# FastLM/CXL-SpecKV

Hardware: AMD Instinct MI355X
Metric: KV blocks/s fetch+decompress (higher is better)
Workload: dtype fp32 (int8 records -> fp16)

## Files before the change

cxl-speckv_amd/csrc/attend_kv.hip:

```cpp
#include "kernels.hpp"
#include "codec_device.hpp"
#include "attend_device.hpp"

namespace speckv {

namespace {

__device__ __forceinline__ uint2 kv_ldg8(const uint8_t* p)
{
    const u32x2 v = __builtin_nontemporal_load(SPECKV_GP(u32x2, p));
    return make_uint2(v.x, v.y);
}
__device__ __forceinline__ uint32_t kv_ldg1(const uint8_t* p) { return *SPECKV_GP(uint8_t, p); }
__device__ __forceinline__ f32x4 kv_ldg_f4(const float* p) { return *SPECKV_GP(f32x4, p); }

}

__global__ __launch_bounds__(256) __attribute__((amdgpu_waves_per_eu(4, 4))) void k_attend_k8v4(AttendArgs a, const AttendKvSide* __restrict__ vside)
{
    const uint32_t lane = threadIdx.x & 63u;
    const uint32_t wave = __builtin_amdgcn_readfirstlane(threadIdx.x >> 6);
    const uint32_t c = lane & 15u, kb = lane >> 4;
    const uint32_t split = a.rows_first ? blockIdx.y : blockIdx.x, by = a.rows_first ? blockIdx.x : blockIdx.y;
    if (a.rows_first && by >= a.rows_real) return;
    const uint32_t hq = a.heads / 4u;
    uint32_t seq = by / hq;
    if (a.order) seq = a.order[seq];
    const uint32_t head = (by % hq) * 4u + wave;
    const uint64_t row = static_cast<uint64_t>(seq) * a.heads + head;
    const AttendSeq sq = a.seqs[seq];
    if (split >= sq.n_splits) {
        if (sq.n_splits == 0u && split == 0u) attend_zero_rows(a.direct_out, a.direct_lse, a.g, row, lane);
        return;
    }
    const AttendKvSide vsd = vside[seq];
    const uint64_t part = sq.part_base + static_cast<uint64_t>(head) * sq.n_splits + split;
    const uint32_t n_pages = sq.n_pages;

    uint32_t qd[8];
    float qscale = 1.0f;
    auto quantise_query = [&]() {
        float xq[32];
        float mx = 0.0f;
        const uint16_t* qsrc = a.q16 + (row * a.g + min(c, a.g - 1u)) * 128u + kb * 16u;
#pragma unroll
        for (int i = 0; i < 4; ++i) {
            const uint4 w = *reinterpret_cast<const uint4*>(qsrc + 8 * (i & 1) + 64 * (i >> 1));
            const uint32_t ws[4] = {w.x, w.y, w.z, w.w};
#pragma unroll
            for (int k = 0; k < 8; ++k) {
                xq[8 * i + k] = static_cast<float>(__builtin_bit_cast(_Float16, static_cast<uint16_t>(ws[k >> 1] >> (16 * (k & 1)))));
                mx = fmaxf(mx, fabsf(xq[8 * i + k]));
            }
        }
        mx = max_over_kb(mx);
        const bool finite = mx < INFINITY;
        const float sc = (mx > 0.0f) ? (finite ? div448_of_f16_value(mx) : mx / 448.0f) : 1.0f;
        const float rcp = finite ? rcp_of_scale(sc) : 0.0f;
        const bool live = c < a.g;
#pragma unroll
        for (int i = 0; i < 8; ++i) {
            float v[4];
#pragma unroll
            for (int k = 0; k < 4; ++k) {
                const float x = xq[4 * i + k];
                const float qt = finite ? __builtin_copysignf(div_by_scale(x, sc, rcp), x) : x / sc;
                v[k] = live ? fminf(fmaxf(qt, -448.0f), 448.0f) : 0.0f;
            }
            int pk = __builtin_amdgcn_cvt_pk_fp8_f32(v[0], v[1], 0, false);
            pk = __builtin_amdgcn_cvt_pk_fp8_f32(v[2], v[3], pk, true);
            qd[i] = static_cast<uint32_t>(pk);
        }
        qscale = (live ? sc : 1.0f) * a.scale_log2e;
    };

    const uint32_t n_tiles = (n_pages + 15u) / 16u;
    const uint32_t t0 = split * sq.tiles_per_split;
    const uint32_t t1 = min(t0 + sq.tiles_per_split, n_tiles);
    float m_run = -INFINITY, l_run = 0.0f;
    f32x4 acc[8];
#pragma unroll
    for (int t = 0; t < 8; ++t) acc[t] = f32x4{0.0f, 0.0f, 0.0f, 0.0f};

    if (t0 < t1) {
        const uint8_t* kp = sq.lin_base + sq.k_first * 2048ull + head * 128u + kb * 16u + (static_cast<uint64_t>(t0) * 32u + c) * 1024u;
        const float* kt = sq.scale_tab + (sq.k_first + static_cast<uint64_t>(t0) * 16u) + 4u * kb;
        const uint8_t* vtile = vsd.v_base + ((vsd.v_first >> 4) + t0) * static_cast<uint64_t>(kMx4TileBytes);
        const uint8_t* vp = vtile + 2u * kb * 1024u + head * 128u + 8u * c;
        const uint8_t* vc = vtile + kMx4CodePlane + 2u * kb * 64u + head * 8u + (c >> 1);

        uint4 kx[2][2];
        uint2 vx[4];
        uint32_t vcode[4];
        f32x4 ks4;
        auto issue_k = [&]() {
#pragma unroll
            for (int b = 0; b < 2; ++b) { kx[b][0] = ldg16(kp + 16384 * b); kx[b][1] = ldg16(kp + 16384 * b + 64); }
            ks4 = kv_ldg_f4(kt);
        };
        auto issue_v = [&]() {
#pragma unroll
            for (int r = 0; r < 4; ++r) vx[r] = kv_ldg8(vp + 1024 * (r & 1) + 8192 * (r >> 1));
#pragma unroll
            for (int r = 0; r < 4; ++r) vcode[r] = kv_ldg1(vc + 64 * (r & 1) + 512 * (r >> 1));
        };
        __builtin_amdgcn_sched_barrier(0);
        issue_k();
        __builtin_amdgcn_sched_barrier(0);
        issue_v();
        __builtin_amdgcn_sched_barrier(0);
        quantise_query();
        __builtin_amdgcn_sched_barrier(0);
        const bool ragged = (n_pages & 15u) != 0u;
#pragma unroll 1
        for (uint32_t tile = t0; tile < t1; ++tile) {
            const uint32_t step = (tile + 1u < t1) ? 1u : 0u;
            float sc[8];
#pragma unroll
            for (int b = 0; b < 2; ++b) {
                const uint32_t kd[8] = {kx[b][0].x, kx[b][0].y, kx[b][0].z, kx[b][0].w, kx[b][1].x, kx[b][1].y, kx[b][1].z, kx[b][1].w};
                f32x4 s = {0.0f, 0.0f, 0.0f, 0.0f};
#pragma unroll
                for (int st = 0; st < 4; ++st)
                    s = __builtin_amdgcn_mfma_f32_16x16x32_fp8_fp8(pack64(kd[2 * st], kd[2 * st + 1]), pack64(qd[2 * st], qd[2 * st + 1]), s, 0, 0, 0);
#pragma unroll
                for (int i = 0; i < 4; ++i) sc[4 * b + i] = s[i] * (ks4[2 * b + (i >> 1)] * qscale);
            }
            if (ragged && tile + 1u == n_tiles) {
#pragma unroll
                for (int r = 0; r < 4; ++r) {
                    const uint32_t pg = tile * 16u + 2u * kb + (r & 1) + 8u * (r >> 1);
                    if (pg >= n_pages) { sc[2 * r] = -INFINITY; sc[2 * r + 1] = -INFINITY; vcode[r] = 0u; }
                }
            }
            __builtin_amdgcn_sched_barrier(0);
            kp += step * 32768u; kt += step * 16u;
            issue_k();
            __builtin_amdgcn_sched_barrier(0);
            float mx = sc[0];
#pragma unroll
            for (int j = 1; j < 8; ++j) mx = fmaxf(mx, sc[j]);
            mx = max_over_kb(mx);
            const float m_new = fmaxf(m_run, mx);
            const float m_use = (m_new == -INFINITY) ? 0.0f : m_new;
            const float f = __builtin_amdgcn_exp2f(m_run - m_use);
            m_run = m_new;
            float psum = 0.0f;
            f16x8 P;
#pragma unroll
            for (int j = 0; j < 8; ++j) {
                const float p = __builtin_amdgcn_exp2f(sc[j] - m_use);
                psum += p;
                P[j] = static_cast<_Float16>(p);
            }
            l_run = l_run * f + psum;
            float vsc[4];
#pragma unroll
            for (int r = 0; r < 4; ++r) vsc[r] = __uint_as_float(vcode[r] << 23);
#define KV_PV(T, WORD, SEL)                                                                                                       \
    {                                                                                                                              \
        const u32x4 vw = {__builtin_bit_cast(uint32_t, __builtin_amdgcn_cvt_scalef32_pk_f16_fp4(vx[0].WORD, vsc[0], SEL)),          \
                          __builtin_bit_cast(uint32_t, __builtin_amdgcn_cvt_scalef32_pk_f16_fp4(vx[1].WORD, vsc[1], SEL)),          \
                          __builtin_bit_cast(uint32_t, __builtin_amdgcn_cvt_scalef32_pk_f16_fp4(vx[2].WORD, vsc[2], SEL)),          \
                          __builtin_bit_cast(uint32_t, __builtin_amdgcn_cvt_scalef32_pk_f16_fp4(vx[3].WORD, vsc[3], SEL))};         \
        acc[T] = __builtin_amdgcn_mfma_f32_16x16x32_f16(__builtin_bit_cast(f16x8, vw), P, acc[T] * f, 0, 0, 0);                     \
    }
            KV_PV(0, x, 0) KV_PV(1, x, 1) KV_PV(2, x, 2) KV_PV(3, x, 3) KV_PV(4, y, 0) KV_PV(5, y, 1) KV_PV(6, y, 2) KV_PV(7, y, 3)
#undef KV_PV
            __builtin_amdgcn_sched_barrier(0);
            vp += step * kMx4TileBytes; vc += step * kMx4TileBytes;
            issue_v();
            __builtin_amdgcn_sched_barrier(0);
        }
    }
    const float l_tot = sum_over_kb(l_run);
    if (sq.n_splits == 1u) {
        if (c < a.g) {
            const float w = l_tot > 0.0f ? 1.0f / l_tot : 0.0f;
            float* dst = a.direct_out + (row * a.g + c) * 128u + 32u * kb;
#pragma unroll
            for (int i = 0; i < 4; ++i) {
                *reinterpret_cast<f32x4*>(dst + 8 * i) = f32x4{acc[0][i], acc[1][i], acc[2][i], acc[3][i]} * w;
                *reinterpret_cast<f32x4*>(dst + 8 * i + 4) = f32x4{acc[4][i], acc[5][i], acc[6][i], acc[7][i]} * w;
            }
            if (a.direct_lse && kb == 0)
                a.direct_lse[row * a.g + c] = l_tot > 0.0f ? (m_run + log2f(l_tot)) * 0.6931471805599453f : -INFINITY;
        }
        return;
    }
    if (kb == 0) {
        a.part_ml[part * 32u + c] = m_run;
        a.part_ml[part * 32u + 16u + c] = l_tot;
    }
    if (c < a.g) {
        float* dst = a.part_acc + (part * 16u + c) * 128u + 32u * kb;
#pragma unroll
        for (int i = 0; i < 4; ++i) {
            *reinterpret_cast<f32x4*>(dst + 8 * i) = f32x4{acc[0][i], acc[1][i], acc[2][i], acc[3][i]};
            *reinterpret_cast<f32x4*>(dst + 8 * i + 4) = f32x4{acc[4][i], acc[5][i], acc[6][i], acc[7][i]};
        }
    }
}

hipError_t launch_attend_k8v4(const AttendArgs& a, const AttendKvSide* d_vside, uint32_t n_seq, bool merge, float* d_out, float* d_lse, hipStream_t s)
{
    if (n_seq == 0) return hipSuccess;
    if (!a.seqs || !d_vside || !a.q16 || a.direct_out != d_out || a.heads % 4u || a.g == 0 || a.g > 16u) return hipErrorInvalidValue;
    AttendArgs ar = a;
    const uint32_t rows = n_seq * (a.heads / 4u), splits = a.n_splits ? a.n_splits : 1u;
    ar.rows_real = rows;
    const dim3 gr = a.rows_first ? dim3(rows | 1u, splits) : dim3(splits, rows);
    hipLaunchKernelGGL(k_attend_k8v4, gr, dim3(256), 0, s, ar, d_vside);
    const hipError_t e = hipGetLastError();
    if (e != hipSuccess || !merge) return e;
    return launch_attend_combine(a, n_seq, d_out, d_lse, s);
}

}
```

cxl-speckv_amd/csrc/tuning.cpp:

```cpp
#include "tuning.hpp"

#include <cstdlib>
#include <cstring>
#include <mutex>

namespace speckv {

namespace {
struct Key { const char* name; const char* env; int32_t Tuning::* field; };
const Key kKeys[] = {
    {"attend_splits", "SPECKV_ATTEND_SPLITS", &Tuning::attend_splits},
    {"attend_tiles_per_split", "SPECKV_ATTEND_TILES_PER_SPLIT", &Tuning::attend_tiles_per_split},
    {"attend_general", "SPECKV_ATTEND_GENERAL", &Tuning::attend_general},
    {"attend_fold_launch", "SPECKV_ATTEND_FOLD_LAUNCH", &Tuning::attend_fold_launch},
    {"attend_layers_loop", "SPECKV_ATTEND_LAYERS_LOOP", &Tuning::attend_layers_loop},
    {"attend_fp8_dma", "SPECKV_ATTEND_FP8_DMA", &Tuning::attend_fp8_dma},
    {"attend_fp8_striped_table", "SPECKV_ATTEND_FP8_STRIPED_TABLE", &Tuning::attend_fp8_striped_table},
    {"attend_int4_striped_wg", "SPECKV_ATTEND_INT4_STRIPED_WG", &Tuning::attend_int4_striped_wg},
    {"attend_fp8_table_regs", "SPECKV_ATTEND_FP8_TABLE_REGS", &Tuning::attend_fp8_table_regs},
    {"attend_stream", "SPECKV_ATTEND_STREAM", &Tuning::attend_stream},
    {"attend_mx4_one_half", "SPECKV_ATTEND_MX4_ONE_HALF", &Tuning::attend_mx4_one_half},
    {"attend_order_as_given", "SPECKV_ATTEND_ORDER_AS_GIVEN", &Tuning::attend_order_as_given},
    {"tc_multipass", "SPECKV_TC_MULTIPASS", &Tuning::tc_multipass},
    {"tc_scan", "SPECKV_TC_SCAN", &Tuning::tc_scan},
    {"tc_no_pre", "SPECKV_TC_NO_PRE", &Tuning::tc_no_pre},
    {"tc_no_split_tiles", "SPECKV_TC_NO_SPLIT_TILES", &Tuning::tc_no_split_tiles},
    {"td_one_pass", "SPECKV_TD_ONE_PASS", &Tuning::td_one_pass},
    {"td_expand_per_element", "SPECKV_TD_EXPAND_PER_ELEMENT", &Tuning::td_expand_per_element},
    {"tc_batch_one_wg", "SPECKV_TC_BATCH_ONE_WG", &Tuning::tc_batch_one_wg},
    {"flush_no_small", "SPECKV_FLUSH_NO_SMALL", &Tuning::flush_no_small},
    {"flush_small_words", "SPECKV_FLUSH_SMALL_WORDS", &Tuning::flush_small_words},
    {"predict_batch_path", "SPECKV_PREDICT_BATCH_PATH", &Tuning::predict_batch_path},
    {"wgs_per_cu", "SPECKV_WGS_PER_CU", &Tuning::wgs_per_cu},
    {"rounds_consecutive", "SPECKV_ROUNDS", &Tuning::rounds_consecutive},
    {"remote_engine", "SPECKV_REMOTE_ENGINE", &Tuning::remote_engine},
    {"copy_min_run_kb", "SPECKV_COPY_MIN_RUN_KB", &Tuning::copy_min_run_kb},
    {"slots_kind_fast", "SPECKV_SLOTS_KIND_FAST", &Tuning::slots_kind_fast},
};
int32_t parse(const char* env_name, const char* v)
{
    if (!strcmp(env_name, "SPECKV_TC_SCAN")) return !strcmp(v, "wg") ? 1 : !strcmp(v, "serial") ? 2 : atoi(v);
    if (!strcmp(env_name, "SPECKV_REMOTE_ENGINE")) return !strcmp(v, "kernel") ? 1 : !strcmp(v, "copy") ? 2 : atoi(v);
    if (!strcmp(env_name, "SPECKV_ROUNDS")) return !strcmp(v, "consecutive") ? 1 : atoi(v);
    if (!*v) return 1;
    const int32_t n = static_cast<int32_t>(atoi(v));
    return (n == 0 && v[0] != '0') ? 1 : n;
}
Tuning g_tuning;
std::once_flag g_once;
}

Tuning& tuning()
{
    std::call_once(g_once, [] {
        for (const Key& k : kKeys)
            if (const char* v = getenv(k.env)) g_tuning.*(k.field) = parse(k.env, v);
    });
    return g_tuning;
}

int tuning_set(const char* key, long long value)
{
    if (!key) return -1;
    Tuning& t = tuning();
    for (const Key& k : kKeys)
        if (!strcmp(k.name, key)) { t.*(k.field) = static_cast<int32_t>(value); return 0; }
    return -1;
}

}
```

cxl-speckv_amd/csrc/tuning.hpp:

```cpp
#pragma once
#include <cstdint>

namespace speckv {

struct Tuning {
    int32_t attend_splits = 0;
    int32_t attend_tiles_per_split = 0;
    int32_t attend_stream = 0;
    int32_t attend_mx4_one_half = 0;
    int32_t attend_order_as_given = 0;
    int32_t attend_general = 0;
    int32_t attend_fp8_table_regs = 0;
    int32_t attend_fp8_dma = 0;
    int32_t attend_fp8_striped_table = 0;
    int32_t attend_int4_striped_wg = 0;
    int32_t attend_layers_loop = 0;
    int32_t attend_fold_launch = 0;
    int32_t tc_multipass = 0;
    int32_t tc_scan = 0;
    int32_t tc_no_pre = 0;
    int32_t tc_no_split_tiles = 0;
    int32_t td_one_pass = 0;
    int32_t td_expand_per_element = 0;
    int32_t tc_batch_one_wg = 0;
    int32_t flush_no_small = 0;
    int32_t flush_small_words = 0;
    int32_t predict_batch_path = 0;
    int32_t wgs_per_cu = 0;
    int32_t rounds_consecutive = 0;
    int32_t remote_engine = 0;
    int32_t copy_min_run_kb = 1024;
    int32_t slots_kind_fast = 0;
};

Tuning& tuning();
int tuning_set(const char* key, long long value);

}
```

Before: 773.5 million.

## Add LDS-DMA double-buffered variant of k8v4 attend kernel and make it default

Adds a new k8v4 attention kernel that streams K, V, scales and codes into per-wave LDS buffers using global_load_lds with swizzled layouts, double-buffered two tiles ahead, and reads them back with explicit waitcnt-controlled ds_reads. The intent is to hide global load latency and reduce VGPR pressure from register-held prefetches. Shared math is factored into helper functions reused by both kernels. The default tuning value (0, tested with >=0) selects the new kernel, which lowers occupancy to 3 waves per EU and relies on hand-counted vmcnt values that could be fragile.

```diff
diff --git a/cxl-speckv_amd/csrc/attend_kv.hip b/cxl-speckv_amd/csrc/attend_kv.hip
--- a/cxl-speckv_amd/csrc/attend_kv.hip
+++ b/cxl-speckv_amd/csrc/attend_kv.hip
@@ -1,18 +1,165 @@
 #include "kernels.hpp"
 #include "codec_device.hpp"
 #include "attend_device.hpp"
+#include "tuning.hpp"
 
 namespace speckv {
 
 namespace {
 
-__device__ __forceinline__ uint2 kv_ldg8(const uint8_t* p)
-{
-    const u32x2 v = __builtin_nontemporal_load(SPECKV_GP(u32x2, p));
-    return make_uint2(v.x, v.y);
-}
+__device__ __forceinline__ u32x2 kv_ldg8(const uint8_t* p) { return __builtin_nontemporal_load(SPECKV_GP(u32x2, p)); }
 __device__ __forceinline__ uint32_t kv_ldg1(const uint8_t* p) { return *SPECKV_GP(uint8_t, p); }
 __device__ __forceinline__ f32x4 kv_ldg_f4(const float* p) { return *SPECKV_GP(f32x4, p); }
+
+__device__ __forceinline__ void kv_quantise_rows(const u32x4 (&w4)[4], bool live, uint32_t (&qd)[8], float& row_scale)
+{
+    float xq[32];
+    float mx = 0.0f;
+#pragma unroll
+    for (int i = 0; i < 4; ++i) {
+        const uint32_t ws[4] = {w4[i].x, w4[i].y, w4[i].z, w4[i].w};
+#pragma unroll
+        for (int k = 0; k < 8; ++k) {
+            xq[8 * i + k] = static_cast<float>(__builtin_bit_cast(_Float16, static_cast<uint16_t>(ws[k >> 1] >> (16 * (k & 1)))));
+            mx = fmaxf(mx, fabsf(xq[8 * i + k]));
+        }
+    }
+    mx = max_over_kb(mx);
+    const bool finite = mx < INFINITY;
+    const float sc = (mx > 0.0f) ? (finite ? div448_of_f16_value(mx) : mx / 448.0f) : 1.0f;
+    const float rcp = finite ? rcp_of_scale(sc) : 0.0f;
+#pragma unroll
+    for (int i = 0; i < 8; ++i) {
+        float v[4];
+#pragma unroll
+        for (int k = 0; k < 4; ++k) {
+            const float x = xq[4 * i + k];
+            const float qt = finite ? __builtin_copysignf(div_by_scale(x, sc, rcp), x) : x / sc;
+            v[k] = live ? fminf(fmaxf(qt, -448.0f), 448.0f) : 0.0f;
+        }
+        int pk = __builtin_amdgcn_cvt_pk_fp8_f32(v[0], v[1], 0, false);
+        pk = __builtin_amdgcn_cvt_pk_fp8_f32(v[2], v[3], pk, true);
+        qd[i] = static_cast<uint32_t>(pk);
+    }
+    row_scale = live ? sc : 1.0f;
+}
+
+__device__ __forceinline__ void kv_store(const AttendArgs& a, uint32_t n_splits, uint64_t row, uint64_t part, uint32_t c, uint32_t kb,
+                                         const f32x4 (&acc)[8], float m_run, float l_run)
+{
+    const float l_tot = sum_over_kb(l_run);
+    if (n_splits == 1u) {
+        if (c < a.g) {
+            const float w = l_tot > 0.0f ? 1.0f / l_tot : 0.0f;
+            float* dst = a.direct_out + (row * a.g + c) * 128u + 32u * kb;
+#pragma unroll
+            for (int i = 0; i < 4; ++i) {
+                *reinterpret_cast<f32x4*>(dst + 8 * i) = f32x4{acc[0][i], acc[1][i], acc[2][i], acc[3][i]} * w;
+                *reinterpret_cast<f32x4*>(dst + 8 * i + 4) = f32x4{acc[4][i], acc[5][i], acc[6][i], acc[7][i]} * w;
+            }
+            if (a.direct_lse && kb == 0)
+                a.direct_lse[row * a.g + c] = l_tot > 0.0f ? (m_run + log2f(l_tot)) * 0.6931471805599453f : -INFINITY;
+        }
+        return;
+    }
+    if (kb == 0) {
+        a.part_ml[part * 32u + c] = m_run;
+        a.part_ml[part * 32u + 16u + c] = l_tot;
+    }
+    if (c < a.g) {
+        float* dst = a.part_acc + (part * 16u + c) * 128u + 32u * kb;
+#pragma unroll
+        for (int i = 0; i < 4; ++i) {
+            *reinterpret_cast<f32x4*>(dst + 8 * i) = f32x4{acc[0][i], acc[1][i], acc[2][i], acc[3][i]};
+            *reinterpret_cast<f32x4*>(dst + 8 * i + 4) = f32x4{acc[4][i], acc[5][i], acc[6][i], acc[7][i]};
+        }
+    }
+}
+
+__device__ __forceinline__ void kv_scores(const uint32_t (&kd)[2][8], const uint32_t (&qd)[8], f32x4 ks4, float qscale, float (&sc)[8])
+{
+#pragma unroll
+    for (int b = 0; b < 2; ++b) {
+        f32x4 s = {0.0f, 0.0f, 0.0f, 0.0f};
+#pragma unroll
+        for (int st = 0; st < 4; ++st)
+            s = __builtin_amdgcn_mfma_f32_16x16x32_fp8_fp8(pack64(kd[b][2 * st], kd[b][2 * st + 1]), pack64(qd[2 * st], qd[2 * st + 1]), s, 0, 0, 0);
+#pragma unroll
+        for (int i = 0; i < 4; ++i) sc[4 * b + i] = s[i] * (ks4[2 * b + (i >> 1)] * qscale);
+    }
+}
+__device__ __forceinline__ void kv_mask_pages(uint32_t tile, uint32_t kb, uint32_t n_pages, float (&sc)[8], uint32_t (&vcode)[4])
+{
+#pragma unroll
+    for (int r = 0; r < 4; ++r) {
+        const uint32_t pg = tile * 16u + 2u * kb + (r & 1) + 8u * (r >> 1);
+        if (pg >= n_pages) { sc[2 * r] = -INFINITY; sc[2 * r + 1] = -INFINITY; vcode[r] = 0u; }
+    }
+}
+__device__ __forceinline__ float kv_softmax(const float (&sc)[8], float& m_run, float& l_run, f16x8& P)
+{
+    float mx = sc[0];
+#pragma unroll
+    for (int j = 1; j < 8; ++j) mx = fmaxf(mx, sc[j]);
+    mx = max_over_kb(mx);
+    const float m_new = fmaxf(m_run, mx);
+    const float m_use = (m_new == -INFINITY) ? 0.0f : m_new;
+    const float f = __builtin_amdgcn_exp2f(m_run - m_use);
+    m_run = m_new;
+    float psum = 0.0f;
+#pragma unroll
+    for (int j = 0; j < 8; ++j) {
+        const float p = __builtin_amdgcn_exp2f(sc[j] - m_use);
+        psum += p;
+        P[j] = static_cast<_Float16>(p);
+    }
+    l_run = l_run * f + psum;
+    return f;
+}
+__device__ __forceinline__ void kv_pv(const u32x2 (&vx)[4], const uint32_t (&vcode)[4], f16x8 P, float f, f32x4 (&acc)[8])
+{
+    float vsc[4];
+#pragma unroll
+    for (int r = 0; r < 4; ++r) vsc[r] = __uint_as_float(vcode[r] << 23);
+#define KV_PV(T, WORD, SEL)                                                                                                       \
+    {                                                                                                                              \
+        const u32x4 vw = {__builtin_bit_cast(uint32_t, __builtin_amdgcn_cvt_scalef32_pk_f16_fp4(vx[0].WORD, vsc[0], SEL)),          \
+                          __builtin_bit_cast(uint32_t, __builtin_amdgcn_cvt_scalef32_pk_f16_fp4(vx[1].WORD, vsc[1], SEL)),          \
+                          __builtin_bit_cast(uint32_t, __builtin_amdgcn_cvt_scalef32_pk_f16_fp4(vx[2].WORD, vsc[2], SEL)),          \
+                          __builtin_bit_cast(uint32_t, __builtin_amdgcn_cvt_scalef32_pk_f16_fp4(vx[3].WORD, vsc[3], SEL))};         \
+        acc[T] = __builtin_amdgcn_mfma_f32_16x16x32_f16(__builtin_bit_cast(f16x8, vw), P, acc[T] * f, 0, 0, 0);                     \
+    }
+    KV_PV(0, x, 0) KV_PV(1, x, 1) KV_PV(2, x, 2) KV_PV(3, x, 3) KV_PV(4, y, 0) KV_PV(5, y, 1) KV_PV(6, y, 2) KV_PV(7, y, 3)
+#undef KV_PV
+}
+
+constexpr uint32_t kKdV = 4096u, kKdS = 6144u, kKdC = kKdS + 64u, kKdBuf = 6400u;
+__device__ __forceinline__ uint32_t kd_row_slot(uint32_t r) { return r ^ ((r >> 2) & 1u); }
+__device__ __forceinline__ uint32_t kd_piece_xor(uint32_t r) { return (r >> 1) & 7u; }
+__device__ __forceinline__ uint32_t kd_page_slot(uint32_t p) { return p ^ ((p >> 1) & 1u); }
+__device__ __forceinline__ void kd_dma16_nt(uint32_t lds_dst, const uint8_t* base, uint32_t voff)
+{
+    uint32_t keep;
+    asm volatile("s_mov_b32 %0, m0\n\ts_mov_b32 m0, %1\n\ts_nop 0\n\tglobal_load_lds_dwordx4 %2, %3 nt\n\ts_mov_b32 m0, %0"
+                 : "=&s"(keep) : "s"(lds_dst), "v"(voff), "s"(base) : "memory");
+}
+__device__ __forceinline__ void kd_take_k(uint32_t rd0, uint32_t rd1, uint32_t rs, uint32_t rc, u32x4 (&k)[4], f32x4& ks, uint32_t (&code)[4])
+{
+    asm volatile("s_waitcnt vmcnt(9)\n\t"
+                 "ds_read_b128 %0, %9\n\tds_read_b128 %1, %10\n\tds_read_b128 %2, %9 offset:2048\n\tds_read_b128 %3, %10 offset:2048\n\t"
+                 "ds_read_b128 %4, %11\n\t"
+                 "ds_read_u8 %5, %12\n\tds_read_u8 %6, %12 offset:8\n\tds_read_u8 %7, %12 offset:64\n\tds_read_u8 %8, %12 offset:72\n\t"
+                 "s_waitcnt lgkmcnt(0)"
+                 : "=&v"(k[0]), "=&v"(k[1]), "=&v"(k[2]), "=&v"(k[3]), "=&v"(ks), "=&v"(code[0]), "=&v"(code[1]), "=&v"(code[2]), "=&v"(code[3])
+                 : "v"(rd0), "v"(rd1), "v"(rs), "v"(rc) : "memory");
+}
+__device__ __forceinline__ void kd_take_v(uint32_t rd0, uint32_t rd1, u32x2 (&v)[4])
+{
+    asm volatile("s_waitcnt vmcnt(12)\n\t"
+                 "ds_read_b64 %0, %4\n\tds_read_b64 %1, %5\n\tds_read_b64 %2, %4 offset:1024\n\tds_read_b64 %3, %5 offset:1024\n\t"
+                 "s_waitcnt lgkmcnt(0)"
+                 : "=&v"(v[0]), "=&v"(v[1]), "=&v"(v[2]), "=&v"(v[3]) : "v"(rd0), "v"(rd1) : "memory");
+}
 
 }
 
@@ -40,38 +187,12 @@
     uint32_t qd[8];
     float qscale = 1.0f;
     auto quantise_query = [&]() {
-        float xq[32];
-        float mx = 0.0f;
         const uint16_t* qsrc = a.q16 + (row * a.g + min(c, a.g - 1u)) * 128u + kb * 16u;
-#pragma unroll
-        for (int i = 0; i < 4; ++i) {
-            const uint4 w = *reinterpret_cast<const uint4*>(qsrc + 8 * (i & 1) + 64 * (i >> 1));
-            const uint32_t ws[4] = {w.x, w.y, w.z, w.w};
-#pragma unroll
-            for (int k = 0; k < 8; ++k) {
-                xq[8 * i + k] = static_cast<float>(__builtin_bit_cast(_Float16, static_cast<uint16_t>(ws[k >> 1] >> (16 * (k & 1)))));
-                mx = fmaxf(mx, fabsf(xq[8 * i + k]));
-            }
-        }
-        mx = max_over_kb(mx);
-        const bool finite = mx < INFINITY;
-        const float sc = (mx > 0.0f) ? (finite ? div448_of_f16_value(mx) : mx / 448.0f) : 1.0f;
-        const float rcp = finite ? rcp_of_scale(sc) : 0.0f;
-        const bool live = c < a.g;
-#pragma unroll
-        for (int i = 0; i < 8; ++i) {
-            float v[4];
-#pragma unroll
-            for (int k = 0; k < 4; ++k) {
-                const float x = xq[4 * i + k];
-                const float qt = finite ? __builtin_copysignf(div_by_scale(x, sc, rcp), x) : x / sc;
-                v[k] = live ? fminf(fmaxf(qt, -448.0f), 448.0f) : 0.0f;
-            }
-            int pk = __builtin_amdgcn_cvt_pk_fp8_f32(v[0], v[1], 0, false);
-            pk = __builtin_amdgcn_cvt_pk_fp8_f32(v[2], v[3], pk, true);
-            qd[i] = static_cast<uint32_t>(pk);
-        }
-        qscale = (live ? sc : 1.0f) * a.scale_log2e;
+        u32x4 w4[4];
+#pragma unroll
+        for (int i = 0; i < 4; ++i) w4[i] = *reinterpret_cast<const u32x4*>(qsrc + 8 * (i & 1) + 64 * (i >> 1));
+        kv_quantise_rows(w4, c < a.g, qd, qscale);
+        qscale *= a.scale_log2e;
     };
 
     const uint32_t n_tiles = (n_pages + 15u) / 16u;
@@ -90,7 +211,7 @@
         const uint8_t* vc = vtile + kMx4CodePlane + 2u * kb * 64u + head * 8u + (c >> 1);
 
         uint4 kx[2][2];
-        uint2 vx[4];
+        u32x2 vx[4];
         uint32_t vcode[4];
         f32x4 ks4;
         auto issue_k = [&]() {
@@ -116,90 +237,134 @@
         for (uint32_t tile = t0; tile < t1; ++tile) {
             const uint32_t step = (tile + 1u < t1) ? 1u : 0u;
             float sc[8];
-#pragma unroll
-            for (int b = 0; b < 2; ++b) {
-                const uint32_t kd[8] = {kx[b][0].x, kx[b][0].y, kx[b][0].z, kx[b][0].w, kx[b][1].x, kx[b][1].y, kx[b][1].z, kx[b][1].w};
-                f32x4 s = {0.0f, 0.0f, 0.0f, 0.0f};
-#pragma unroll
-                for (int st = 0; st < 4; ++st)
-                    s = __builtin_amdgcn_mfma_f32_16x16x32_fp8_fp8(pack64(kd[2 * st], kd[2 * st + 1]), pack64(qd[2 * st], qd[2 * st + 1]), s, 0, 0, 0);
-#pragma unroll
-                for (int i = 0; i < 4; ++i) sc[4 * b + i] = s[i] * (ks4[2 * b + (i >> 1)] * qscale);
-            }
-            if (ragged && tile + 1u == n_tiles) {
-#pragma unroll
-                for (int r = 0; r < 4; ++r) {
-                    const uint32_t pg = tile * 16u + 2u * kb + (r & 1) + 8u * (r >> 1);
-                    if (pg >= n_pages) { sc[2 * r] = -INFINITY; sc[2 * r + 1] = -INFINITY; vcode[r] = 0u; }
-                }
-            }
+            const uint32_t kd[2][8] = {{kx[0][0].x, kx[0][0].y, kx[0][0].z, kx[0][0].w, kx[0][1].x, kx[0][1].y, kx[0][1].z, kx[0][1].w},
+                                       {kx[1][0].x, kx[1][0].y, kx[1][0].z, kx[1][0].w, kx[1][1].x, kx[1][1].y, kx[1][1].z, kx[1][1].w}};
+            kv_scores(kd, qd, ks4, qscale, sc);
+            if (ragged && tile + 1u == n_tiles) kv_mask_pages(tile, kb, n_pages, sc, vcode);
             __builtin_amdgcn_sched_barrier(0);
             kp += step * 32768u; kt += step * 16u;
             issue_k();
             __builtin_amdgcn_sched_barrier(0);
-            float mx = sc[0];
-#pragma unroll
-            for (int j = 1; j < 8; ++j) mx = fmaxf(mx, sc[j]);
-            mx = max_over_kb(mx);
-            const float m_new = fmaxf(m_run, mx);
-            const float m_use = (m_new == -INFINITY) ? 0.0f : m_new;
-            const float f = __builtin_amdgcn_exp2f(m_run - m_use);
-            m_run = m_new;
-            float psum = 0.0f;
             f16x8 P;
-#pragma unroll
-            for (int j = 0; j < 8; ++j) {
-                const float p = __builtin_amdgcn_exp2f(sc[j] - m_use);
-                psum += p;
-                P[j] = static_cast<_Float16>(p);
-            }
-            l_run = l_run * f + psum;
-            float vsc[4];
-#pragma unroll
-            for (int r = 0; r < 4; ++r) vsc[r] = __uint_as_float(vcode[r] << 23);
-#define KV_PV(T, WORD, SEL)                                                                                                       \
-    {                                                                                                                              \
-        const u32x4 vw = {__builtin_bit_cast(uint32_t, __builtin_amdgcn_cvt_scalef32_pk_f16_fp4(vx[0].WORD, vsc[0], SEL)),          \
-                          __builtin_bit_cast(uint32_t, __builtin_amdgcn_cvt_scalef32_pk_f16_fp4(vx[1].WORD, vsc[1], SEL)),          \
-                          __builtin_bit_cast(uint32_t, __builtin_amdgcn_cvt_scalef32_pk_f16_fp4(vx[2].WORD, vsc[2], SEL)),          \
-                          __builtin_bit_cast(uint32_t, __builtin_amdgcn_cvt_scalef32_pk_f16_fp4(vx[3].WORD, vsc[3], SEL))};         \
-        acc[T] = __builtin_amdgcn_mfma_f32_16x16x32_f16(__builtin_bit_cast(f16x8, vw), P, acc[T] * f, 0, 0, 0);                     \
-    }
-            KV_PV(0, x, 0) KV_PV(1, x, 1) KV_PV(2, x, 2) KV_PV(3, x, 3) KV_PV(4, y, 0) KV_PV(5, y, 1) KV_PV(6, y, 2) KV_PV(7, y, 3)
-#undef KV_PV
+            const float f = kv_softmax(sc, m_run, l_run, P);
+            kv_pv(vx, vcode, P, f, acc);
             __builtin_amdgcn_sched_barrier(0);
             vp += step * kMx4TileBytes; vc += step * kMx4TileBytes;
             issue_v();
             __builtin_amdgcn_sched_barrier(0);
         }
     }
-    const float l_tot = sum_over_kb(l_run);
-    if (sq.n_splits == 1u) {
-        if (c < a.g) {
-            const float w = l_tot > 0.0f ? 1.0f / l_tot : 0.0f;
-            float* dst = a.direct_out + (row * a.g + c) * 128u + 32u * kb;
-#pragma unroll
-            for (int i = 0; i < 4; ++i) {
-                *reinterpret_cast<f32x4*>(dst + 8 * i) = f32x4{acc[0][i], acc[1][i], acc[2][i], acc[3][i]} * w;
-                *reinterpret_cast<f32x4*>(dst + 8 * i + 4) = f32x4{acc[4][i], acc[5][i], acc[6][i], acc[7][i]} * w;
-            }
-            if (a.direct_lse && kb == 0)
-                a.direct_lse[row * a.g + c] = l_tot > 0.0f ? (m_run + log2f(l_tot)) * 0.6931471805599453f : -INFINITY;
-        }
+    kv_store(a, sq.n_splits, row, part, c, kb, acc, m_run, l_run);
+}
+
+__global__ __launch_bounds__(256) __attribute__((amdgpu_waves_per_eu(3, 3))) void k_attend_k8v4_dma(AttendArgs a, const AttendKvSide* __restrict__ vside)
+{
+    __shared__ __attribute__((aligned(16))) uint8_t lds[4][2 * kKdBuf];
+    const uint32_t lane = threadIdx.x & 63u;
+    const uint32_t wave = __builtin_amdgcn_readfirstlane(threadIdx.x >> 6);
+    const uint32_t c = lane & 15u, kb = lane >> 4;
+    const uint32_t split = a.rows_first ? blockIdx.y : blockIdx.x, by = a.rows_first ? blockIdx.x : blockIdx.y;
+    if (a.rows_first && by >= a.rows_real) return;
+    const uint32_t hq = a.heads / 4u;
+    uint32_t seq = by / hq;
+    if (a.order) seq = a.order[seq];
+    const uint32_t head = (by % hq) * 4u + wave;
+    const uint64_t row = static_cast<uint64_t>(seq) * a.heads + head;
+    const AttendSeq sq = a.seqs[seq];
+    if (split >= sq.n_splits) {
+        if (sq.n_splits == 0u && split == 0u) attend_zero_rows(a.direct_out, a.direct_lse, a.g, row, lane);
         return;
     }
-    if (kb == 0) {
-        a.part_ml[part * 32u + c] = m_run;
-        a.part_ml[part * 32u + 16u + c] = l_tot;
-    }
-    if (c < a.g) {
-        float* dst = a.part_acc + (part * 16u + c) * 128u + 32u * kb;
-#pragma unroll
-        for (int i = 0; i < 4; ++i) {
-            *reinterpret_cast<f32x4*>(dst + 8 * i) = f32x4{acc[0][i], acc[1][i], acc[2][i], acc[3][i]};
-            *reinterpret_cast<f32x4*>(dst + 8 * i + 4) = f32x4{acc[4][i], acc[5][i], acc[6][i], acc[7][i]};
-        }
-    }
+    const AttendKvSide vsd = vside[seq];
+    const uint64_t part = sq.part_base + static_cast<uint64_t>(head) * sq.n_splits + split;
+    const uint32_t n_pages = sq.n_pages;
+    const uint32_t n_tiles = (n_pages + 15u) / 16u;
+    const uint32_t t0 = __builtin_amdgcn_readfirstlane(split * sq.tiles_per_split);
+    const uint32_t t1 = __builtin_amdgcn_readfirstlane(min(t0 + sq.tiles_per_split, n_tiles));
+    float m_run = -INFINITY, l_run = 0.0f;
+    f32x4 acc[8];
+#pragma unroll
+    for (int t = 0; t < 8; ++t) acc[t] = f32x4{0.0f, 0.0f, 0.0f, 0.0f};
+
+    if (t0 < t1) {
+        const uint8_t* kreg = uniform_ptr(sq.lin_base + sq.k_first * 2048ull + head * 128u);
+        const uint8_t* vtile0 = vsd.v_base + (vsd.v_first >> 4) * static_cast<uint64_t>(kMx4TileBytes);
+        const uint8_t* vreg = uniform_ptr(vtile0 + head * 128u);
+        uint32_t gk[4], gv[2];
+#pragma unroll
+        for (uint32_t i = 0; i < 4; ++i) {
+            const uint32_t r = kd_row_slot(8u * i + (lane >> 3));
+            gk[i] = r * 1024u + (((lane & 7u) ^ kd_piece_xor(r)) * 16u);
+        }
+#pragma unroll
+        for (uint32_t i = 0; i < 2; ++i) gv[i] = kd_page_slot(8u * i + (lane >> 3)) * 1024u + (lane & 7u) * 16u;
+        const uint32_t cl = (lane - 16u) & 31u;
+        const uint8_t* sc_src = lane < 16u ? reinterpret_cast<const uint8_t*>(sq.scale_tab + sq.k_first + lane)
+                                           : vtile0 + kMx4CodePlane + (cl >> 1) * 64u + head * 8u + (cl & 1u) * 4u;
+        const uint32_t sc_step = lane < 16u ? 64u : kMx4TileBytes;
+        const uint32_t lbase = __builtin_amdgcn_readfirstlane(static_cast<uint32_t>(reinterpret_cast<uintptr_t>(&lds[wave][0])));
+        const uint32_t last = t1 - 1u;
+        auto issue_k = [&](uint32_t tt, uint32_t buf) {
+            const uint32_t tc = min(tt, last);
+            const uint8_t* src = kreg + static_cast<uint64_t>(tc) * 32768u;
+            const uint32_t dst = lbase + buf * kKdBuf;
+#pragma unroll
+            for (uint32_t i = 0; i < 4; ++i) kd_dma16_nt(dst + 1024u * i, src, gk[i]);
+            if (lane < 48u) dma4v(dst + kKdS, sc_src + static_cast<uint64_t>(tc) * sc_step);
+        };
+        auto issue_v = [&](uint32_t tt, uint32_t buf) {
+            const uint8_t* src = vreg + static_cast<uint64_t>(min(tt, last)) * kMx4TileBytes;
+            const uint32_t dst = lbase + buf * kKdBuf + kKdV;
+#pragma unroll
+            for (uint32_t i = 0; i < 2; ++i) kd_dma16_nt(dst + 1024u * i, src, gv[i]);
+        };
+        const uint32_t kslot = kd_row_slot(c), kxr = kd_piece_xor(c);
+        const uint32_t rdk0 = lbase + kslot * 128u + ((kb ^ kxr) * 16u);
+        const uint32_t rdk1 = lbase + kslot * 128u + (((4u + kb) ^ kxr) * 16u);
+        const uint32_t rsc = lbase + kKdS + kb * 16u;
+        const uint32_t rcd = lbase + kKdC + kb * 16u + (c >> 1);
+        const uint32_t rdv0 = lbase + kKdV + kd_page_slot(2u * kb) * 128u + 8u * c;
+        const uint32_t rdv1 = lbase + kKdV + kd_page_slot(2u * kb + 1u) * 128u + 8u * c;
+        issue_k(t0, 0u);
+        u32x4 qw[4];
+        {
+            const uint16_t* qsrc = a.q16 + (row * a.g + min(c, a.g - 1u)) * 128u + kb * 16u;
+            asm volatile("global_load_dwordx4 %0, %4, off\n\tglobal_load_dwordx4 %1, %4, off offset:16\n\t"
+                         "global_load_dwordx4 %2, %4, off offset:128\n\tglobal_load_dwordx4 %3, %4, off offset:144"
+                         : "=&v"(qw[0]), "=&v"(qw[1]), "=&v"(qw[2]), "=&v"(qw[3]) : "v"(qsrc) : "memory");
+        }
+        issue_v(t0, 0u);
+        issue_k(t0 + 1u, 1u);
+        issue_v(t0 + 1u, 1u);
+        asm volatile("s_waitcnt vmcnt(9)" : "+v"(qw[0]), "+v"(qw[1]), "+v"(qw[2]), "+v"(qw[3]) :: "memory");
+        uint32_t qd[8];
+        float qscale;
+        kv_quantise_rows(qw, c < a.g, qd, qscale);
+        qscale *= a.scale_log2e;
+        const bool ragged = (n_pages & 15u) != 0u;
+#pragma unroll 1
+        for (uint32_t tile = t0; tile < t1; ++tile) {
+            const uint32_t buf = (tile - t0) & 1u, bo = buf * kKdBuf;
+            u32x4 kx[4];
+            f32x4 ks4;
+            uint32_t vcode[4];
+            kd_take_k(rdk0 + bo, rdk1 + bo, rsc + bo, rcd + bo, kx, ks4, vcode);
+            issue_k(tile + 2u, buf);
+            float sc[8];
+            const uint32_t kd[2][8] = {{kx[0].x, kx[0].y, kx[0].z, kx[0].w, kx[1].x, kx[1].y, kx[1].z, kx[1].w},
+                                       {kx[2].x, kx[2].y, kx[2].z, kx[2].w, kx[3].x, kx[3].y, kx[3].z, kx[3].w}};
+            kv_scores(kd, qd, ks4, qscale, sc);
+            if (ragged && tile + 1u == n_tiles) kv_mask_pages(tile, kb, n_pages, sc, vcode);
+            f16x8 P;
+            const float f = kv_softmax(sc, m_run, l_run, P);
+            u32x2 vx[4];
+            kd_take_v(rdv0 + bo, rdv1 + bo, vx);
+            issue_v(tile + 2u, buf);
+            kv_pv(vx, vcode, P, f, acc);
+        }
+        asm volatile("s_waitcnt vmcnt(0)" ::: "memory");
+    }
+    kv_store(a, sq.n_splits, row, part, c, kb, acc, m_run, l_run);
 }
 
 hipError_t launch_attend_k8v4(const AttendArgs& a, const AttendKvSide* d_vside, uint32_t n_seq, bool merge, float* d_out, float* d_lse, hipStream_t s)
@@ -210,7 +375,8 @@
     const uint32_t rows = n_seq * (a.heads / 4u), splits = a.n_splits ? a.n_splits : 1u;
     ar.rows_real = rows;
     const dim3 gr = a.rows_first ? dim3(rows | 1u, splits) : dim3(splits, rows);
-    hipLaunchKernelGGL(k_attend_k8v4, gr, dim3(256), 0, s, ar, d_vside);
+    if (tuning().attend_k8v4_dma >= 0) hipLaunchKernelGGL(k_attend_k8v4_dma, gr, dim3(256), 0, s, ar, d_vside);
+    else hipLaunchKernelGGL(k_attend_k8v4, gr, dim3(256), 0, s, ar, d_vside);
     const hipError_t e = hipGetLastError();
     if (e != hipSuccess || !merge) return e;
     return launch_attend_combine(a, n_seq, d_out, d_lse, s);
diff --git a/cxl-speckv_amd/csrc/tuning.cpp b/cxl-speckv_amd/csrc/tuning.cpp
--- a/cxl-speckv_amd/csrc/tuning.cpp
+++ b/cxl-speckv_amd/csrc/tuning.cpp
@@ -15,6 +15,7 @@
     {"attend_fold_launch", "SPECKV_ATTEND_FOLD_LAUNCH", &Tuning::attend_fold_launch},
     {"attend_layers_loop", "SPECKV_ATTEND_LAYERS_LOOP", &Tuning::attend_layers_loop},
     {"attend_fp8_dma", "SPECKV_ATTEND_FP8_DMA", &Tuning::attend_fp8_dma},
+    {"attend_k8v4_dma", "SPECKV_ATTEND_K8V4_DMA", &Tuning::attend_k8v4_dma},
     {"attend_fp8_striped_table", "SPECKV_ATTEND_FP8_STRIPED_TABLE", &Tuning::attend_fp8_striped_table},
     {"attend_int4_striped_wg", "SPECKV_ATTEND_INT4_STRIPED_WG", &Tuning::attend_int4_striped_wg},
     {"attend_fp8_table_regs", "SPECKV_ATTEND_FP8_TABLE_REGS", &Tuning::attend_fp8_table_regs},
diff --git a/cxl-speckv_amd/csrc/tuning.hpp b/cxl-speckv_amd/csrc/tuning.hpp
--- a/cxl-speckv_amd/csrc/tuning.hpp
+++ b/cxl-speckv_amd/csrc/tuning.hpp
@@ -12,6 +12,7 @@
     int32_t attend_general = 0;
     int32_t attend_fp8_table_regs = 0;
     int32_t attend_fp8_dma = 0;
+    int32_t attend_k8v4_dma = 0;
     int32_t attend_fp8_striped_table = 0;
     int32_t attend_int4_striped_wg = 0;
     int32_t attend_layers_loop = 0;
```

Result: no change. 772.8 million (-0.1%).
